# YuliangXiu/ICON

Measured on AMD Instinct MI355X. Metric: query-points/sec at 256^3 grid, higher is better.
Workload: dtype f32 via 3x f16 split MFMA (22-bit operands, f32 accumulate)

## Files before the change

### icon_amd/csrc/fused_f16x3.hip

```cpp
#pragma clang fp contract(off)

#include "geom_device.h"
#include "batch_device.h"
#include "mlp_f16x3_device.h"
#include "mlp_plain_device.h"

#include <algorithm>
#include <mutex>

namespace icon {

constexpr int kTilePts = kF16Pts;
constexpr int kXsOff = kSideOff + 4352;
constexpr int kFusedLds = kXsOff + kTilePts * kXRow * 4;

struct SignSrc {
    int mode;
    const int8_t *list;
    const int64_t *k_dev;
    int64_t k_host, rank_offset;
    const int8_t *gathered;
    int64_t stride;
    int world, rank;
    const int64_t *seg;
// ... 159 lines not shown
    const int planes = zb - za;
    if ((int)blockIdx.x < row_wgs) {
        const int64_t row = (int64_t)blockIdx.x * 256 + threadIdx.x;
        if (row >= (int64_t)planes * res) return;
        const int iy = (int)(row % res), iz = za + (int)(row / res);
        float *o = out + ((int64_t)(iz - z0) * res + iy) * res;
        o[0] = 0.0f; o[res - 1] = 0.0f;
        return;
    }
    const int f = ((int)blockIdx.x - row_wgs) * 4 + (int)(threadIdx.x >> 6);
    const int lane = threadIdx.x & 63;
    int iy, iz;
    if (f < 2 * planes) { iz = za + (f >> 1); iy = (f & 1) ? res - 1 : 0; }
    else {
        const int g = f - 2 * planes;
        const bool has0 = za == 0, has1 = zb == res;
        const int pl = g / res;
        if (pl >= (has0 ? 1 : 0) + (has1 ? 1 : 0)) return;
        iz = (pl == 0 && has0) ? 0 : res - 1;
        iy = g % res;
    }
    float *o = out + ((int64_t)(iz - z0) * res + iy) * res;
    for (int x = lane; x < res; x += 64) o[x] = 0.0f;
}

__device__ __forceinline__ float sign_at(const SignSrc &sg, int64_t mm)
{
    if (sg.mode == kSignSeg) {
        int r = 0;
        int64_t base = 0;
        for (int q = 1; q < sg.world; ++q) {
            const int64_t o = sg.seg[q];
            const bool ge = mm >= o;
            r += ge ? 1 : 0;
            base = ge ? o : base;
        }
        const int64_t e = mm - base;
        const uint32_t byte = (uint8_t)sg.gathered[(int64_t)r * sg.stride + 8 + (e >> 2)];
        return (float)((int)((byte >> (2 * (int)(e & 3))) & 3u) - 1);
    }
    return (float)sg.list[mm];
}

__device__ __forceinline__ int64_t lattice_item(const FusedGeom &G, int64_t q, int &ix, int &iy, int &iz)
{
    const uint32_t nx = (uint32_t)G.nx, qq = (uint32_t)q;
    const uint32_t r = qq / nx, lx = qq - r * nx, lz = r / nx, ly = r - lz * nx;
    ix = G.off + (int)lx; iy = G.off + (int)ly; iz = G.zs + (int)lz;
    return ((int64_t)(iz - G.z0) * G.res + iy) * G.res + ix;
}

__device__ __forceinline__ int64_t uniform64(int64_t v)
{
    const uint32_t lo = (uint32_t)__builtin_amdgcn_readfirstlane((int)(uint32_t)v);
    const uint32_t hi = (uint32_t)__builtin_amdgcn_readfirstlane((int)(uint32_t)((uint64_t)v >> 32));
    return (int64_t)(((uint64_t)hi << 32) | lo);
}

__device__ __forceinline__ void icon_row(const FusedGeom &G, const MeshDev &m, const FeatDev &f, f3 p, int64_t i, float *xrow, int64_t K, int64_t rank0)
{
    const uint32_t code = G.code8[i];
    Nearest nr;
    nr.slot = near_slot_of(G.near, i); nr.face = 0;
    nr.d2 = (code & kCodeOutlier) ? 0.0f : near_d2(G.near, i);
    const SdfOut o = sdf_attrs(m, p, nr, (code & kCodeInside) != 0);
    float s = o.sdf;
    f3 cmv = o.cm;
    if (code & kCodeOutlier) {
        s = (float)((int)((code >> kCodeSignShift) & 3u) - 1);
        if (G.cmap_local) cmv = mk3(s, s, s);
        else if (K > 0 && (f.smpl_mask & kSmplCmap)) {
            const int64_t blk = i >> 8;
            const int g = (int)(i >> 6) & 3;
            const unsigned long long *mk = G.grp_mask + blk * 4;
            int before = __popcll(mk[g] & ((1ull << (i & 63)) - 1ull));
            if (g > 0) before += __popcll(mk[0]);
            if (g > 1) before += __popcll(mk[1]);
            if (g > 2) before += __popcll(mk[2]);
            const int64_t jr = rank0 + G.block_offsets[blk] + before;
            float c3[3];
#pragma unroll
            for (int k = 0; k < 3; ++k) {
                int64_t mm = 3 * jr + k;
                if (mm >= K) mm -= K;
                if (mm >= K) mm -= K;
                c3[k] = sign_at(G.sg, mm);
            }
            cmv = mk3(c3[0], c3[1], c3[2]);
        }
    }
    gather_planes_dyn(f, (f.n_select == 2 && o.vis == 0.0f) ? 1 : 0, p.x, p.y, xrow);
    int hh = f.csel;
    xrow[hh++] = s;
    if (f.smpl_mask & kSmplCmap) { xrow[hh] = cmv.x; xrow[hh + 1] = cmv.y; xrow[hh + 2] = cmv.z; hh += 3; }
    if (f.smpl_mask & kSmplNorm) { xrow[hh] = o.nrm.x; xrow[hh + 1] = o.nrm.y; xrow[hh + 2] = o.nrm.z; }
    xrow[kCodeSlot] = __int_as_float((int)(code & kCodeInCube));
}

template <int PRIOR, Src SRC>
__device__ __forceinline__ void build_row(const FusedGeom &G, const BatchDev &bd, int64_t q, float *xrow, int64_t K, int64_t rank0)
{
    f3 p;
    int64_t i;
    const int64_t b = SRC == Src::Batch ? q / bd.n : 0;
    if (SRC == Src::Lattice) {
        int ix, iy, iz;
        i = lattice_item(G, q, ix, iy, iz);
        p = lattice_world(G.res, ix, iy, iz);
    } else {
        i = q;
        p = project(SRC == Src::Batch ? batch_calib(bd, b) : resolve_calib(G.cal), mk3(G.pts[3 * i], G.pts[3 * i + 1], G.pts[3 * i + 2]));
    }
    const FeatDev f = SRC == Src::Batch ? batch_feat(G.f, bd, b) : G.f;
    if (PRIOR == ICON_PRIOR_ICON) {
        icon_row(G, SRC == Src::Batch ? bd.meshes[b] : G.m, f, p, i, xrow, K, rank0);
    } else {
        gather_planes_dyn(f, 0, p.x, p.y, xrow);
        const int hh = f.csel;
        if (PRIOR == ICON_PRIOR_PAMIR) {
            float v[8];
            if (f.vpad == 8) gather_volume<2>(f, p.x, p.y, p.z, v); else gather_volume<1>(f, p.x, p.y, p.z, v);
#pragma unroll
            for (int k = 0; k < 8; ++k) if (k < f.Cv) xrow[hh + k] = v[k];
        } else {
            xrow[hh] = p.z;
        }
        xrow[kCodeSlot] = __int_as_float((int)in_cube_bit(p));
    }
}

__device__ __forceinline__ void sign_list_extent(const FusedGeom &G, int64_t &K, int64_t &rank0)
{
    K = 0; rank0 = 0;
    if (G.cmap_local) return;
    if (G.sg.mode == kSignSelf) K = *G.sg.k_dev;
    else if (G.sg.mode == kSignGlobal) { K = G.sg.k_host; rank0 = G.sg.rank_offset; }
    else if (G.sg.mode == kSignSeg) { K = G.sg.seg[G.sg.world]; rank0 = G.sg.seg[G.sg.rank]; }
}

template <int PRIOR, Src SRC, bool SMALL = false>
__global__ __launch_bounds__(kF16Block, 2) void k_fused_f16x3(FusedGeom G, float *__restrict__ out, MlpF16Dev w, BatchDev bd)
{
    extern __shared__ __attribute__((aligned(16))) char smem[];
    const int lane0 = threadIdx.x & 63, wave0 = __builtin_amdgcn_readfirstlane(threadIdx.x >> 6);
    float *Xs = reinterpret_cast<float *>(smem + kXsOff);
    if (G.clock && threadIdx.x == 0) {
        if (blockIdx.x == 0) wg_stamp(G.clock);
        if (blockIdx.x < kMaxProfGrid) wg_stamp(G.clock + 4 + kWgRec * blockIdx.x);
    }

    issue_units(w.image, smem + kW0Off, kW0Bytes / 1024, wave0, lane0);
    float *side = reinterpret_cast<float *>(smem + kSideOff);
    for (int i = threadIdx.x; i < kSideFloats; i += kF16Block) side[i] = w.side[i];
    const float *sb0 = side, *sb1 = side + 512, *sb2 = side + 768, *sw3 = side + kW3Float;
    int64_t K = 0, rank0 = 0;
    if (PRIOR == ICON_PRIOR_ICON) sign_list_extent(G, K, rank0);
    K = uniform64(K); rank0 = uniform64(rank0);

    if (SRC != Src::Batch && G.n_dev) { G.N = *G.n_dev; if (G.N <= 0) return; }
    const int tp = (SMALL && G.N <= (int64_t)(kTilePts / 2) * gridDim.x) ? kTilePts / 2 : kTilePts;
    const int ntiles = (int)((G.N + tp - 1) / tp);
    const bool stealing = !SMALL && G.steal != nullptr;
    const int per = ntiles / (int)gridDim.x, rem = ntiles % (int)gridDim.x;
    int tile = (int)blockIdx.x * per + min((int)blockIdx.x, rem);
    int tile_end = tile + (stealing ? min(G.steal_static, per) : per + ((int)blockIdx.x < rem ? 1 : 0));
    tile = __builtin_amdgcn_readfirstlane(tile);
    tile_end = __builtin_amdgcn_readfirstlane(tile_end);
    volatile int *pool = reinterpret_cast<volatile int *>(smem + kPoolOff);
    if (!SMALL) {
        if (threadIdx.x == 0) {
            pool[kPoolPer] = per; pool[kPoolRem] = rem; pool[kPoolStatic] = G.steal_static; pool[kPoolGroup] = G.steal_grp;
            pool[kPoolNGrp] = G.steal_ngrp; pool[kPoolGrid] = (int)gridDim.x; pool[kPoolDone] = 0; pool[kPoolMask] = 0; pool[kPoolNext] = -1;
            if (stealing && tile >= tile_end) pool_draw(G.steal, pool);
        }
        __syncthreads();
        if (stealing && tile >= tile_end) {
            const int word = __builtin_amdgcn_readfirstlane(pool[kPoolNext]);
            __syncthreads();
            if (word >= 0) { tile = word & ((1 << kPoolLenShift) - 1); tile_end = tile + (word >> kPoolLenShift); }
        }
    }
    if (tile < tile_end) issue_chunk(w.image, smem, 0, wave0, lane0);

    for (int nb = -1; tile < tile_end;) {
        int tid = threadIdx.x;
        asm volatile("" : "+v"(tid));
        const int lane = tid & 63, wave = __builtin_amdgcn_readfirstlane(tid >> 6);
        const int r = lane & 15, g = lane >> 4;
        const int t = tid;
        const bool draw = !SMALL && stealing && tile + 1 == tile_end;
        if (!SMALL && draw && t == 256) pool_draw(G.steal, pool);
        const bool worker = t < tp;
        int64_t q = (int64_t)tile * tp + (worker ? t : 0);
        if (q >= G.N) q = G.N - 1;
        if (worker) build_row<PRIOR, SRC>(G, bd, q, Xs + t * kXRow, K, rank0);
        __syncthreads();

        nb = (!SMALL && draw) ? __builtin_amdgcn_readfirstlane(pool[kPoolNext]) : -1;
        if (!SMALL && tid == 0) pool[kPoolDone] = pool[kPoolDone] + 1;
        const bool more = tile + 1 < tile_end || nb >= 0;
        if (SMALL && wave >= (tp >> 5)) {
            for (int c = 0; c < 16; ++c) {
                issue_chunk(w.image, smem + ((c + 1) & 1) * kBufBytes, c + 1, wave, lane);
                ICON_CHUNK_BARRIER();
            }
            issue_chunk(w.image, smem + kBufBytes, 17, wave, lane);
            ICON_CHUNK_BARRIER();
            issue_chunk(w.image, smem, 18, wave, lane);
            ICON_CHUNK_BARRIER();
            issue_chunk(w.image, smem + kBufBytes, 19, wave, lane);
            ICON_CHUNK_BARRIER();
            if (more) issue_chunk(w.image, smem, 0, wave, lane);
            ++tile;
            continue;
        }
        const int pt = wave * 32 + 16 * (g & 1) + r;
        half8 xb[2];
        const float tail = load_x(Xs + (wave * 32 + r) * kXRow + 8 * (g & 1), Xs + (wave * 32 + 16 + r) * kXRow + 8 * (g & 1), sw3, w.c0, g, xb);
        float maskf = (__float_as_int(Xs[pt * kXRow + kCodeSlot]) & (int)kCodeInCube) ? 1.0f : 0.0f;
        asm volatile("" : "+v"(maskf));

        f32x4 acc1[16][2];
#pragma unroll
        for (int m = 0; m < 16; ++m) acc1[m][0] = acc1[m][1] = *reinterpret_cast<const f32x4 *>(sb1 + m * 16 + 4 * g);
        half8 bh[2], bl[2];
        const LeakyK k0{w.inv0, w.p0, w.q0}, k1{w.inv1, w.p1, w.q1};
        {
            f32x4 h0[2][2];
            l0_tiles(smem + kW0Off, sb0, 0, xb, g, lane, h0);
            activate_split(h0[0][0], h0[0][1], h0[1][0], h0[1][1], k0, bh, bl);
        }
        f32x4 acc2[8][2];
        for (int c = 0; c < 15; ++c) {
            l01_chunk<false>(smem + (c & 1) * kBufBytes, smem + ((c + 1) & 1) * kBufBytes, smem + kW0Off, sb0, w.image, c, acc1, xb,
                             k0, g, lane, wave, bh, bl);
            ICON_CHUNK_BARRIER();
        }
        l01_chunk<true>(smem + kBufBytes, smem, smem + kW0Off, sb0, w.image, 15, acc1, xb, k0, g, lane, wave, bh, bl);
        ICON_CHUNK_BARRIER();
#pragma unroll
        for (int m2 = 0; m2 < 8; ++m2) acc2[m2][0] = acc2[m2][1] = *reinterpret_cast<const f32x4 *>(sb2 + m2 * 16 + 4 * g);
        activate_split(acc1[0][0], acc1[1][0], acc1[0][1], acc1[1][1], k1, bh, bl);
        l2_chunk<0>(smem, smem + kBufBytes, w.image, acc1, acc2, xb, k1, g, lane, wave, bh, bl);
        ICON_CHUNK_BARRIER();
        l2_chunk<1>(smem + kBufBytes, smem, w.image, acc1, acc2, xb, k1, g, lane, wave, bh, bl);
        ICON_CHUNK_BARRIER();
        l2_chunk<2>(smem, smem + kBufBytes, w.image, acc1, acc2, xb, k1, g, lane, wave, bh, bl);
        ICON_CHUNK_BARRIER();
        l2_chunk<3>(smem + kBufBytes, smem, w.image, acc1, acc2, xb, k1, g, lane, wave, bh, bl, more ? 0 : -1);

        float y2[2];
        {
            int tid_3 = threadIdx.x;
            asm volatile("" : "+v"(tid_3), "+v"(acc2[0][0]));
            l3_sum(sw3, acc2, tail, LeakyK{w.inv2, w.p2, w.q2}, w.b3, (tid_3 >> 4) & 3, y2);
        }
        int tid_o = threadIdx.x;
        asm volatile("" : "+v"(tid_o), "+v"(y2[0]), "+v"(y2[1]));
        const int g_o = (tid_o >> 4) & 3, pt_o = (tid_o >> 6) * 32 + 16 * (g_o & 1) + (tid_o & 15);
        const float y = apply_last_op(g_o == 0 ? y2[0] : y2[1], w.last_op);
        const int64_t oq = (int64_t)tile * tp + pt_o;
        if (g_o < 2 && oq < G.N) {
            int ix, iy, iz;
            out[SRC == Src::Lattice ? lattice_item(G, oq, ix, iy, iz) : ((SRC == Src::Points && G.out_map) ? (int64_t)G.out_map[oq] : oq)] = masked_result(y, maskf != 0.0f, w.flag);
        }
        if (!SMALL && nb >= 0) {
            tile = nb & ((1 << kPoolLenShift) - 1);
            tile_end = tile + (nb >> kPoolLenShift);
        } else ++tile;
    }
    if (!SMALL && stealing && threadIdx.x == 0) {
        __threadfence();
        if (atomicAdd(G.steal + 8, 1u) == gridDim.x - 1)
            for (int k = 0; k < 9; ++k) atomicExch(G.steal + k, 0u);
    }
    if (G.clock && threadIdx.x == 0 && blockIdx.x < kMaxProfGrid) {
        if (blockIdx.x == 0) wg_stamp(G.clock + 2);
        unsigned long long *rec = G.clock + 4 + kWgRec * blockIdx.x;
        wg_stamp(rec + 2);
        unsigned xcc, hw;
        asm volatile("s_getreg_b32 %0, hwreg(HW_REG_XCC_ID)" : "=s"(xcc));
        asm volatile("s_getreg_b32 %0, hwreg(HW_REG_HW_ID)" : "=s"(hw));
        rec[4] = ((unsigned long long)xcc << 32) | hw;
        rec[5] = SMALL ? 0ull : (unsigned long long)pool[kPoolDone];
    }
}

template <int PRIOR, Src SRC>
__global__ __launch_bounds__(64) void k_rescue_fused(FusedGeom G, float *__restrict__ out, MlpPlain P, const int *flag, int always, BatchDev bd)
{
    __shared__ float s[kPlainLds];
    if (!always && *flag == 0) return;
    if (SRC != Src::Batch && G.n_dev) G.N = *G.n_dev;
    const int lane = threadIdx.x;
    int64_t K = 0, rank0 = 0;
    if (PRIOR == ICON_PRIOR_ICON) sign_list_extent(G, K, rank0);
    for (int64_t base = (int64_t)blockIdx.x * 64; base < G.N; base += (int64_t)gridDim.x * 64) {
        const int64_t q = base + lane;
        int ix, iy, iz;
        const int64_t o = q < G.N ? (SRC == Src::Lattice ? lattice_item(G, q, ix, iy, iz) : ((SRC == Src::Points && G.out_map) ? (int64_t)G.out_map[q] : q)) : 0;
        const float v = q < G.N ? out[o] : 0.0f;
        unsigned long long todo = __ballot(not_finite(v));
        while (todo) {
            const int b = __ffsll((long long)todo) - 1;
            todo &= todo - 1;
            if (lane == b) {
                float row[kXRow];
#pragma unroll
                for (int k = 0; k < kXRow; ++k) row[k] = 0.0f;
                build_row<PRIOR, SRC>(G, bd, q, row, K, rank0);
#pragma unroll
                for (int k = 0; k < kXRow; ++k) s[k] = k < P.c0 ? row[k] : 0.0f;
            }
            const float y = mlp_plain_wave(P, s, lane);
            if (lane == b) out[o] = y;
            __builtin_amdgcn_wave_barrier();
        }
    }
}

__global__ void k_seg_offsets(const int8_t *__restrict__ gathered, int64_t stride, int world, int64_t *__restrict__ seg)
{
    if (threadIdx.x != 0 || blockIdx.x != 0) return;
    int64_t a = 0;
    for (int r = 0; r < world; ++r) { seg[r] = a; a += *reinterpret_cast<const int64_t *>(gathered + (int64_t)r * stride); }
    seg[world] = a;
}

int launch_sign(const icon_mesh *mesh, const Calib &cal, int res, int z0, const float *d_points, int64_t N, float sdf_clip,
                const icon_work *work, bool lattice, hipStream_t st, const BatchDev *bd)
{
    const int64_t nb = (N + 255) / 256;
    ICON_ARG(nb > 0 && nb < (1ll << 31), "too many workgroups for one launch");
    const float far_box2 = far_box_dist2(sdf_clip);
    if (lattice) hipLaunchKernelGGL(k_sign<true>, dim3((unsigned)nb), dim3(256), 0, st, mesh->dev, cal, res, z0, d_points, N, sdf_clip,
                                    work->d_row_count, work->d_row_slots, work_near(work, mesh), work->d_code8, work->d_block_counts,
                                    (unsigned long long *)work->d_grp_mask, far_box2, (const int *)nullptr, work->d_flag);
    else if (bd)
        hipLaunchKernelGGL(k_sign_wide<true>, dim3((unsigned)nb), dim3(1024), 0, st, MeshDev{}, Calib{}, d_points, N, sdf_clip, work_near(work, mesh), work->d_code8,
                           work->d_block_counts, (unsigned long long *)work->d_grp_mask, far_box2, (const int *)nullptr, work->d_flag, *bd);
    else if (work->q_n_dev || N <= 262144)
        hipLaunchKernelGGL(k_sign_wide<false>, dim3((unsigned)nb), dim3(1024), 0, st, mesh->dev, cal, d_points, N, sdf_clip, work_near(work, mesh), work->d_code8,
                           work->d_block_counts, (unsigned long long *)work->d_grp_mask, far_box2, work->q_n_dev, work->d_flag, BatchDev{});
    else hipLaunchKernelGGL(k_sign<false>, dim3((unsigned)nb), dim3(256), 0, st, mesh->dev, cal, res, z0, d_points, N, sdf_clip,
                            (const int32_t *)nullptr, (const int32_t *)nullptr, work_near(work, mesh), work->d_code8, work->d_block_counts,
                            (unsigned long long *)work->d_grp_mask, far_box2, work->q_n_dev, work->d_flag);
    ICON_HIP(hipGetLastError());
    work->flag_clean = work->d_flag != nullptr;
    return ICON_OK;
}

namespace {
constexpr int kMaxDevices = 64, kMaxKernelIds = 16;
std::mutex g_dev_mutex;
int g_n_cu[kMaxDevices];
bool g_attr_set[kMaxKernelIds][kMaxDevices];
}

int device_cu_count(int *n_cu)
{
    int dev = 0;
    ICON_HIP(hipGetDevice(&dev));
    ICON_ARG(dev >= 0 && dev < kMaxDevices, "device index out of range");
    std::lock_guard<std::mutex> lk(g_dev_mutex);
    if (!g_n_cu[dev]) {
        int n = 0;
        ICON_HIP(hipDeviceGetAttribute(&n, hipDeviceAttributeMultiprocessorCount, dev));
        g_n_cu[dev] = n > 0 ? n : 256;
    }
    *n_cu = g_n_cu[dev];
    return ICON_OK;
}

int once_per_device(int kernel_id, const std::function<hipError_t()> &set)
{
    int dev = 0;
    if (hipGetDevice(&dev) != hipSuccess || dev < 0 || dev >= kMaxDevices || kernel_id < 0 || kernel_id >= kMaxKernelIds) {
        const hipError_t e = set();
        return e == hipSuccess ? ICON_OK : fail(ICON_ERR_HIP, std::string("hipFuncSetAttribute: ") + hipGetErrorString(e));
    }
    std::lock_guard<std::mutex> lk(g_dev_mutex);
    if (g_attr_set[kernel_id][dev]) return ICON_OK;
    const hipError_t e = set();
    if (e != hipSuccess) return fail(ICON_ERR_HIP, std::string("hipFuncSetAttribute: ") + hipGetErrorString(e));
    g_attr_set[kernel_id][dev] = true;
    return ICON_OK;
}

int launch_fused_f16x3(const icon_mesh *mesh, const icon_feat *feat, const icon_mlp *mlp, int prior, const Calib &cal,
                       const LatticeMap &L, int za, int zb, const float *d_points, int64_t N, float sdf_clip, int cmap_local,
                       const icon_work *work, const FusedSigns &fs, float *d_occ, bool lattice, hipStream_t st, const BatchDev *bd)
{
    FusedGeom G{};
    if (mesh) G.m = mesh->dev;
    G.f = feat->dev; G.cal = cal; G.pts = d_points; G.sdf_clip = sdf_clip; G.cmap_local = cmap_local;
    if (lattice) {
        const int zs = std::max(za, L.off), ze = std::min(zb, L.res - L.off);
        if (L.off) {
            const int64_t rows = (int64_t)(zb - za) * L.res;
            const int row_wgs = (int)((rows + 255) / 256);
            const int64_t face_rows = 2 * (int64_t)(zb - za) + (int64_t)((za == 0 ? 1 : 0) + (zb == L.res ? 1 : 0)) * L.res;
            if (rows > 0) hipLaunchKernelGGL(k_shell_zero, dim3((unsigned)(row_wgs + (face_rows + 3) / 4)), dim3(256), 0, st, d_occ, L.res, L.z0, za, zb, row_wgs);
// ... 80 lines not shown
```

### icon_amd/csrc/mlp_f16x3.hip

```cpp
#include "mlp_f16x3_device.h"

#include <cmath>
#include <cstring>

namespace icon {

template <bool MASK>
__global__ __launch_bounds__(kF16Block, 2) void k_mlp_f16x3(const float *__restrict__ X, int64_t N, float *__restrict__ out, MlpF16Dev w)
{
    extern __shared__ __attribute__((aligned(16))) char smem[];
    const int lane = threadIdx.x & 63, wave = __builtin_amdgcn_readfirstlane(threadIdx.x >> 6);
    const int r = lane & 15, g = lane >> 4;
    const int64_t base = ((int64_t)blockIdx.x * (kF16Block / 64) + wave) * 32;
    const int64_t pi0 = min(base + r, N - 1), pi1 = min(base + 16 + r, N - 1);
    const int64_t po = (g & 1) ? pi1 : pi0;

    issue_units(w.image, smem + kW0Off, kW0Bytes / 1024, wave, lane);
    float *side = reinterpret_cast<float *>(smem + kSideOff);
    for (int i = threadIdx.x; i < kSideFloats; i += kF16Block) side[i] = w.side[i];
    const float *sb0 = side, *sb1 = side + 512, *sb2 = side + 768, *sw3 = side + kW3Float;

    float maskf = 1.0f;
    if (MASK) {
        const uint32_t code = (uint32_t)__float_as_int(X[po * kXRow + kCodeSlot]);
        maskf = (code & kCodeInCube) ? 1.0f : 0.0f;
        asm volatile("" : "+v"(maskf));
    }
    issue_chunk(w.image, smem, 0, wave, lane);
    __syncthreads();
    half8 xb[2];
    const float tail = load_x(X + pi0 * kXRow + 8 * (g & 1), X + pi1 * kXRow + 8 * (g & 1), sw3, w.c0, g, xb);

    f32x4 acc1[16][2];
#pragma unroll
    for (int m = 0; m < 16; ++m) acc1[m][0] = acc1[m][1] = *reinterpret_cast<const f32x4 *>(sb1 + m * 16 + 4 * g);

    half8 bh[2], bl[2];
    const LeakyK k0{w.inv0, w.p0, w.q0}, k1{w.inv1, w.p1, w.q1};
    {
        f32x4 h0[2][2];
        l0_tiles(smem + kW0Off, sb0, 0, xb, g, lane, h0);
        activate_split(h0[0][0], h0[0][1], h0[1][0], h0[1][1], k0, bh, bl);
    }
    for (int c = 0; c < 15; ++c) {
        l01_chunk<false>(smem + (c & 1) * kBufBytes, smem + ((c + 1) & 1) * kBufBytes, smem + kW0Off, sb0, w.image, c, acc1, xb,
                         k0, g, lane, wave, bh, bl);
        ICON_CHUNK_BARRIER();
    }
    l01_chunk<true>(smem + kBufBytes, smem, smem + kW0Off, sb0, w.image, 15, acc1, xb, k0, g, lane, wave, bh, bl);
    ICON_CHUNK_BARRIER();

    f32x4 acc2[8][2];
#pragma unroll
    for (int m2 = 0; m2 < 8; ++m2) acc2[m2][0] = acc2[m2][1] = *reinterpret_cast<const f32x4 *>(sb2 + m2 * 16 + 4 * g);
    activate_split(acc1[0][0], acc1[1][0], acc1[0][1], acc1[1][1], k1, bh, bl);
    l2_chunk<0>(smem, smem + kBufBytes, w.image, acc1, acc2, xb, k1, g, lane, wave, bh, bl);
    ICON_CHUNK_BARRIER();
    l2_chunk<1>(smem + kBufBytes, smem, w.image, acc1, acc2, xb, k1, g, lane, wave, bh, bl);
    ICON_CHUNK_BARRIER();
    l2_chunk<2>(smem, smem + kBufBytes, w.image, acc1, acc2, xb, k1, g, lane, wave, bh, bl);
    ICON_CHUNK_BARRIER();
    l2_chunk<3>(smem + kBufBytes, smem, w.image, acc1, acc2, xb, k1, g, lane, wave, bh, bl);

    float y2[2];
    {
        int tid_3 = threadIdx.x;
        asm volatile("" : "+v"(tid_3), "+v"(acc2[0][0]));
        l3_sum(sw3, acc2, tail, LeakyK{w.inv2, w.p2, w.q2}, w.b3, (tid_3 >> 4) & 3, y2);
    }
    int tid_o = threadIdx.x;
    asm volatile("" : "+v"(tid_o), "+v"(y2[0]), "+v"(y2[1]));
    const int g_o = (tid_o >> 4) & 3;
    const int64_t o = ((int64_t)blockIdx.x * (kF16Block / 64) + (tid_o >> 6)) * 32 + 16 * g_o + (tid_o & 15);
    const float y = apply_last_op(g_o == 0 ? y2[0] : y2[1], w.last_op);
    if (g_o < 2 && o < N) out[o] = masked_result(y, MASK ? maskf != 0.0f : true, w.flag);
}

uint16_t f32_to_f16_rtn(float f)
{
    uint32_t x; memcpy(&x, &f, 4);
    const uint32_t sign = (x >> 16) & 0x8000u;
    x &= 0x7fffffffu;
    if (x >= 0x7f800000u) return (uint16_t)(sign | 0x7c00u | (x > 0x7f800000u ? 0x200u : 0));
    if (x >= 0x477ff000u) return (uint16_t)(sign | 0x7c00u);
    if (x < 0x33000001u) return (uint16_t)sign;
    int e = (int)(x >> 23) - 127;
    uint32_t m = (x & 0x7fffffu) | 0x800000u;
    int shift;
    if (e < -14) { shift = 13 + (-14 - e); e = -15; } else shift = 13;
    uint32_t r = m >> shift;
    const uint32_t rem = m & ((1u << shift) - 1), half = 1u << (shift - 1);
    if (rem > half || (rem == half && (r & 1))) ++r;
    uint32_t out = (e == -15) ? r : (((uint32_t)(e + 15) << 10) + (r - 0x400u));
    return (uint16_t)(sign | out);
}

float f16_to_f32(uint16_t h)
{
    const uint32_t sign = (uint32_t)(h & 0x8000u) << 16;
    const int e = (h >> 10) & 31;
    const uint32_t m = h & 0x3ffu;
    float v;
    if (e == 0) v = std::ldexp((float)m, -24);
    else if (e == 31) v = m ? NAN : INFINITY;
    else v = std::ldexp((float)(m | 0x400u), e - 25);
    return sign ? -v : v;
}

float pick_scale(const std::vector<float> &W)
{
    float mx = 0.f;
    for (float v : W) mx = std::max(mx, std::fabs(v));
    if (!(mx > 0.f) || !std::isfinite(mx)) return 1.0f;
    int e = (int)std::floor(std::log2(8192.0 / (double)mx));
    e = std::min(std::max(e, -60), 60);
    return std::ldexp(1.0f, e);
}

float activation_scale(const std::vector<float> &W, const std::vector<float> &B, int cout, int cin, int n_used, const std::vector<double> &in_ms,
                       std::vector<double> &out_ms)
{
    out_ms.assign(cout, 0.0);
    double acc = 0.0;
    for (int c = 0; c < cout; ++c) {
        double s = (double)B[c] * B[c];
        for (int k = 0; k < n_used; ++k) s += (double)W[(size_t)c * cin + k] * W[(size_t)c * cin + k] * in_ms[k];
        out_ms[c] = s; acc += s;
    }
    const double typical = std::sqrt(acc / std::max(cout, 1));
    if (!(typical > 0.0) || !std::isfinite(typical)) return 1.0f;
    int e = (int)std::lround(std::log2(16.0 / typical));
    e = std::min(std::max(e, -60), 60);
    return std::ldexp(1.0f, e);
}

void mlp_pack_f16x3_host(int c0, const std::vector<std::vector<float>> &W, const std::vector<std::vector<float>> &B,
                         std::vector<uint16_t> &img, std::vector<float> &side, float inv[3], float scales[5])
{
    std::vector<double> ms_in(c0, 1.0), ms0, ms1;
    const float A0 = activation_scale(W[0], B[0], 512, c0, c0, ms_in, ms0);
    std::vector<float> W1(W[1]);
    for (float &v : W1) v /= A0;
    const float A1 = activation_scale(W[1], B[1], 256, 512, 512, ms0, ms1);
    const int ci2_ = 256 + c0;
    std::vector<float> W2(W[2]);
    for (int c = 0; c < 128; ++c)
        for (int k = 0; k < 256; ++k) W2[(size_t)c * ci2_ + k] /= A1;
    const float s0 = pick_scale(W[0]), s1 = pick_scale(W1), s2 = pick_scale(W2);
    img.assign(kImageBytes / 2, 0);
    auto sigma = [](int k) { const int g = k >> 3, e = k & 7; return e < 4 ? 4 * g + e : 16 + 4 * g + (e - 4); };
    auto put = [&](size_t at, size_t lo_step, float wv, float scale) {
        const float ws = wv * scale;
        const uint16_t hi = f32_to_f16_rtn(ws);
        img[at] = hi;
        img[at + lo_step] = f32_to_f16_rtn(ws - f16_to_f32(hi));
    };
    const int ci2 = 256 + c0;
    parallel_for(64, [&](int lane) {
        const int r = lane & 15, g = lane >> 4;
        for (int e = 0; e < 8; ++e) {
            const int ch = sigma(8 * g + e);
            const size_t col = (size_t)lane * 8 + e;
            for (int c = 0; c < 16; ++c)
                for (int mm = 0; mm < 16; ++mm)
                    put(((size_t)chunk_offset(c) + 2 * mm) * 512 + col, 512, W1[(size_t)(16 * mm + r) * 512 + 32 * c + ch], s1);
            for (int q = 0; q < 4; ++q)
                for (int mm = 0; mm < 2; ++mm)
                    for (int m2 = 0; m2 < 8; ++m2)
                        put(((size_t)chunk_offset(16 + q) + (mm * 8 + m2) * 2) * 512 + col, 512,
                            W2[(size_t)(16 * m2 + r) * ci2 + 32 * (2 * q + mm) + ch], s2);
        }
    });
    for (int g1 = 0; g1 < 2; ++g1)
        for (int r = 0; r < 16; ++r)
            for (int e = 0; e < 8; ++e) {
                const int k = 8 * g1 + e;
                const size_t col = (size_t)(g1 * 16 + r) * 8 + e;
                for (int ct = 0; ct < 32; ++ct)
                    put((size_t)ct * 512 + col, 256, k < c0 ? W[0][(size_t)(16 * ct + r) * c0 + k] : 0.f, s0);
                for (int m2 = 0; m2 < 8; ++m2)
                    put(((size_t)chunk_offset(16) + 32 + m2) * 512 + col, 256, k < c0 ? W2[(size_t)(16 * m2 + r) * ci2 + 256 + k] : 0.f, s2);
            }
    side.assign(kSideFloats, 0.f);
    float *b0 = side.data(), *b1 = b0 + 512, *b2 = b1 + 256, *w3 = side.data() + kW3Float;
    for (int c = 0; c < 512; ++c) b0[c] = B[0][c] * s0;
    for (int c = 0; c < 256; ++c) b1[c] = B[1][c] * s1;
    for (int c = 0; c < 128; ++c) b2[c] = B[2][c] * s2;
    for (int g = 0; g < 4; ++g) {
        for (int m2 = 0; m2 < 8; ++m2)
            for (int j = 0; j < 4; ++j) w3[g * kW3Stride + 4 * m2 + j] = W[3][16 * m2 + 4 * g + j];
        for (int s = 0; s < 8; ++s) w3[g * kW3Stride + 32 + s] = (s + 8 * (g & 1) < c0) ? W[3][128 + s + 8 * (g & 1)] : 0.f;
    }
    inv[0] = A0 / s0; inv[1] = A1 / s1; inv[2] = 1.0f / s2;
    scales[0] = s0; scales[1] = s1; scales[2] = s2; scales[3] = A0; scales[4] = A1;
}

int mlp_pack_f16x3(icon_mlp *m, const std::vector<std::vector<float>> &W, const std::vector<std::vector<float>> &B,
                   hipStream_t st)
{
    std::vector<uint16_t> img;
    std::vector<float> side;
    float scales[5];
    mlp_pack_f16x3_host(m->c0, W, B, img, side, m->f16_inv, scales);
    const size_t side_bytes = side.size() * sizeof(float);
    ICON_HIP(hipMalloc((void **)&m->d_f16, kImageBytes + side_bytes));
    ICON_HIP(hipMemcpyAsync(m->d_f16, img.data(), kImageBytes, hipMemcpyHostToDevice, st));
    ICON_HIP(hipMemcpyAsync(m->d_f16 + kImageBytes, side.data(), side_bytes, hipMemcpyHostToDevice, st));
    ICON_HIP(hipStreamSynchronize(st));
    return ICON_OK;
}

int mlp_launch_f16x3(const icon_mlp *mlp, const float *d_x, int64_t N, float *d_out, bool mask, hipStream_t st)
{
    if (N <= 0) return ICON_OK;
    MlpF16Dev w;
// ... 41 lines not shown
```

### icon_amd/csrc/mlp_f16x3_device.h

```cpp
#pragma once
#include "common.h"

namespace icon {

typedef float f32x4 __attribute__((ext_vector_type(4)));
typedef _Float16 half8 __attribute__((ext_vector_type(8)));
typedef __fp16 fp16x2 __attribute__((ext_vector_type(2)));
typedef __attribute__((address_space(1))) const void gvoid_t;
typedef __attribute__((address_space(3))) void lvoid_t;

constexpr int kF16Block = 512;
constexpr int kF16Pts = (kF16Block / 64) * 32;
constexpr int kBufBytes = 40 * 1024;
constexpr int kW3Stride = 40;
constexpr int kW3Float = 512 + 256 + 128;
constexpr int kZeroFloat = kW3Float + 4 * kW3Stride;
constexpr int kSideFloats = kZeroFloat + 4;
constexpr int kW0Off = 2 * kBufBytes;
constexpr int kW0Bytes = 32 * 1024;
constexpr int kSideOff = kW0Off + kW0Bytes;
constexpr int kLdsBytes = kSideOff + 4352;
constexpr int kZeroFromW0 = kSideOff + kZeroFloat * 4 - kW0Off;
constexpr int kZeroFromBuf0 = kSideOff + kZeroFloat * 4;
static_assert(kSideFloats * 4 <= 4352 && kZeroFromW0 % 16 == 0, "side arrays");

__host__ __device__ constexpr int chunk_units(int k) { return k == 16 ? 40 : 32; }
__host__ __device__ constexpr int chunk_offset(int k) { return 32 + 32 * k + (k > 16 ? 8 : 0); }
constexpr size_t kImageBytes = (size_t)(32 + 19 * 32 + 40) * 1024;

struct MlpF16Dev {
    const char *image;
    const float *side;
    float b3;
    float inv0, inv1, inv2;
    float p0, q0, p1, q1, p2, q2;
    int c0;
    int last_op;
    int *flag;
};

__device__ __forceinline__ float masked_result(float y, bool in_cube, int *flag)
{
    if (in_cube && not_finite(y)) *flag = 1;
    return in_cube ? y : 0.0f;
}

__device__ __forceinline__ fp16x2 residual_pair(fp16x2 hh, float v0, float v1)
{
    const int hb = __builtin_bit_cast(int, hh);
    int lb;
    asm("v_fma_mixlo_f16 %0, %1, -1.0, %2 op_sel_hi:[1,0,0]" : "=v"(lb) : "v"(hb), "v"(v0));
    asm("v_fma_mixhi_f16 %0, %1, -1.0, %2 op_sel:[1,0,0] op_sel_hi:[1,0,0]" : "+v"(lb) : "v"(hb), "v"(v1));
    return __builtin_bit_cast(fp16x2, lb);
}

__device__ __forceinline__ void split8(const float *v, half8 &hi, half8 &lo)
{
#pragma unroll
    for (int q = 0; q < 4; ++q) {
        const fp16x2 h = __builtin_amdgcn_cvt_pkrtz(v[2 * q], v[2 * q + 1]);
        const fp16x2 l = residual_pair(h, v[2 * q], v[2 * q + 1]);
        hi[2 * q] = (_Float16)h[0]; hi[2 * q + 1] = (_Float16)h[1];
        lo[2 * q] = (_Float16)l[0]; lo[2 * q + 1] = (_Float16)l[1];
    }
}

#ifndef ICON_ACT_EXACT
#define ICON_ACT_EXACT 0
#endif
struct LeakyK { float inv, p, q; };
__device__ __forceinline__ float leaky_scaled(float a, const LeakyK &k)
{
#if ICON_ACT_EXACT
    const float x = a * k.inv;
    return fmaxf(x, 0.01f * x);
#else
    return fmaf(fabsf(a), k.q, k.p * a);
#endif
}

#define MFMA32(a, b, c) __builtin_amdgcn_mfma_f32_16x16x32_f16((a), (b), (c), 0, 0, 0)

__device__ __forceinline__ half8 lds_op(const char *buf, int slot, int lane)
{
    return *reinterpret_cast<const half8 *>(buf + slot * 1024 + lane * 16);
}

#define ICON_CHUNK_BARRIER() __syncthreads()


__device__ __forceinline__ void issue_units(const char *src, char *buf, int units, int wave, int lane)
{
    for (int u = wave; u < units; u += kF16Block / 64)
        __builtin_amdgcn_global_load_lds((gvoid_t *)(src + u * 1024 + lane * 16), (lvoid_t *)(buf + u * 1024), 16, 0, 0);
}
__device__ __forceinline__ void issue_chunk(const char *image, char *buf, int k, int wave, int lane)
{
    issue_units(image + (size_t)chunk_offset(k) * 1024, buf, chunk_units(k), wave, lane);
}


#define GROUP6(ACC, M, AH, AL, BH, BL)                                                              \
    ACC[M][0] = MFMA32(AH, BH[0], ACC[M][0]); ACC[M][1] = MFMA32(AH, BH[1], ACC[M][1]);             \
    ACC[M][0] = MFMA32(AH, BL[0], ACC[M][0]); ACC[M][1] = MFMA32(AH, BL[1], ACC[M][1]);             \
    ACC[M][0] = MFMA32(AL, BH[0], ACC[M][0]); ACC[M][1] = MFMA32(AL, BH[1], ACC[M][1]);

__device__ __forceinline__ float load_x(const float *row0, const float *row1, const float *__restrict__ sw3, int c0, int g, half8 (&xb)[2])
{
    float tail = 0.0f;
#pragma unroll
    for (int b = 0; b < 2; ++b) {
        const float4 *q = reinterpret_cast<const float4 *>(b ? row1 : row0);
        const float4 u = q[0], v = q[1];
        float x[8] = {u.x, u.y, u.z, u.w, v.x, v.y, v.z, v.w};
#pragma unroll
        for (int s = 0; s < 8; ++s) x[s] = (s + 8 * (g & 1) < c0) ? x[s] : 0.0f;
        half8 hi, lo;
        split8(x, hi, lo);
        xb[b] = g < 2 ? hi : lo;
        float t = 0.0f;
#pragma unroll
        for (int s = 0; s < 8; ++s) t = fmaf(sw3[g * kW3Stride + 32 + s], x[s], t);
        tail = (g >> 1) == b ? t : tail;
    }
    asm volatile("" : "+v"(tail));
    return tail;
}

__device__ __forceinline__ void raw_operands(const char *__restrict__ base, int tile, int zero_off, int g, int lane, half8 &a1, half8 &a2)
{
    const int col = (lane & 31) * 16;
    const int lo_off = g < 2 ? 512 + col : zero_off, lo_mul = g < 2 ? 1024 : 0;
    a1 = *reinterpret_cast<const half8 *>(base + tile * 1024 + col);
    a2 = *reinterpret_cast<const half8 *>(base + lo_off + tile * lo_mul);
}

__device__ __forceinline__ void l0_tiles(const char *__restrict__ W0, const float *__restrict__ sb0, int c, const half8 (&xb)[2],
                                         int g, int lane, f32x4 (&h0)[2][2])
{
#pragma unroll
    for (int t = 0; t < 2; ++t) {
        const f32x4 bias = *reinterpret_cast<const f32x4 *>(sb0 + (2 * c + t) * 16 + 4 * g);
        half8 a1, a2;
        raw_operands(W0, 2 * c + t, kZeroFromW0, g, lane, a1, a2);
        h0[0][t] = MFMA32(a1, xb[0], bias); h0[1][t] = MFMA32(a1, xb[1], bias);
        h0[0][t] = MFMA32(a2, xb[0], h0[0][t]); h0[1][t] = MFMA32(a2, xb[1], h0[1][t]);
    }
}

__device__ __forceinline__ void act_part(const f32x4 &ta0, const f32x4 &tb0, const f32x4 &ta1, const f32x4 &tb1, int k, const LeakyK &inv,
                                         half8 (&nh)[2], half8 (&nl)[2])
{
    const int b = k >> 2, q = k & 3, j0 = (q & 1) * 2;
    const f32x4 &src = b ? (q >> 1 ? tb1 : ta1) : (q >> 1 ? tb0 : ta0);
    const float v0 = leaky_scaled(src[j0], inv), v1 = leaky_scaled(src[j0 + 1], inv);
    fp16x2 hh = __builtin_amdgcn_cvt_pkrtz(v0, v1);
    fp16x2 ll = residual_pair(hh, v0, v1);
    int hb = __builtin_bit_cast(int, hh), lb = __builtin_bit_cast(int, ll);
    asm volatile("" : "+v"(hb), "+v"(lb));
    hh = __builtin_bit_cast(fp16x2, hb); ll = __builtin_bit_cast(fp16x2, lb);
    nh[b][2 * q] = (_Float16)hh[0]; nh[b][2 * q + 1] = (_Float16)hh[1];
    nl[b][2 * q] = (_Float16)ll[0]; nl[b][2 * q + 1] = (_Float16)ll[1];
}

__device__ __forceinline__ void activate_split(const f32x4 &ta0, const f32x4 &tb0, const f32x4 &ta1, const f32x4 &tb1, const LeakyK &inv,
                                               half8 (&bh)[2], half8 (&bl)[2])
{
#pragma unroll
    for (int k = 0; k < 8; ++k) act_part(ta0, tb0, ta1, tb1, k, inv, bh, bl);
}

template <bool LAST>
__device__ __forceinline__ void l01_chunk(const char *__restrict__ L, char *__restrict__ nxt, const char *__restrict__ W0,
                                          const float *__restrict__ sb0, const char *image, int c, f32x4 (&acc1)[16][2],
                                          const half8 (&xb)[2], const LeakyK &inv0, int g4, int lane, int wave,
                                          half8 (&bh)[2], half8 (&bl)[2])
{
    issue_chunk(image, nxt, c + 1, wave, lane);
    f32x4 h0n[2][2];
    if (!LAST) l0_tiles(W0, sb0, c + 1, xb, g4, lane, h0n);
    half8 nh[2], nl[2];
    half8 a[2][2];
    a[0][0] = lds_op(L, 0, lane); a[0][1] = lds_op(L, 1, lane);
    __builtin_amdgcn_sched_barrier(0);
#pragma unroll
    for (int t = 0; t < 16; ++t) {
        if (t + 1 < 16) { a[(t + 1) & 1][0] = lds_op(L, 2 * t + 2, lane); a[(t + 1) & 1][1] = lds_op(L, 2 * t + 3, lane); }
        GROUP6(acc1, t, a[t & 1][0], a[t & 1][1], bh, bl)
        if (!LAST && (t & 1)) act_part(h0n[0][0], h0n[0][1], h0n[1][0], h0n[1][1], t >> 1, inv0, nh, nl);
        __builtin_amdgcn_sched_barrier(0);
    }
    if (!LAST) { bh[0] = nh[0]; bh[1] = nh[1]; bl[0] = nl[0]; bl[1] = nl[1]; }
}

template <int Q>
__device__ __forceinline__ void l2_chunk(const char *__restrict__ L, char *__restrict__ nxt, const char *image,
                                         f32x4 (&acc1)[16][2], f32x4 (&acc2)[8][2], const half8 (&xb)[2], const LeakyK &inv1,
                                         int g4, int lane, int wave, half8 (&bh)[2], half8 (&bl)[2], int next_chunk = (Q < 3) ? 17 + Q : -1)
{
    if (next_chunk >= 0) issue_chunk(image, nxt, next_chunk, wave, lane);
    if (Q == 0) {
#pragma unroll
        for (int m2 = 0; m2 < 8; ++m2) {
            half8 a1, a2;
            raw_operands(L, 32 + m2, kZeroFromBuf0, g4, lane, a1, a2);
            acc2[m2][0] = MFMA32(a1, xb[0], acc2[m2][0]); acc2[m2][1] = MFMA32(a1, xb[1], acc2[m2][1]);
            acc2[m2][0] = MFMA32(a2, xb[0], acc2[m2][0]); acc2[m2][1] = MFMA32(a2, xb[1], acc2[m2][1]);
        }
        __builtin_amdgcn_sched_barrier(0);
    }
#pragma unroll
    for (int mm = 0; mm < 2; ++mm) {
        constexpr int kLast = 7;
        const int kk = 2 * Q + mm, n = kk < kLast ? 2 * kk + 2 : 0;
        half8 nh[2], nl[2];
        half8 a[2][2];
        a[0][0] = lds_op(L, mm * 16, lane); a[0][1] = lds_op(L, mm * 16 + 1, lane);
        __builtin_amdgcn_sched_barrier(0);
#pragma unroll
        for (int t = 0; t < 8; ++t) {
            if (t + 1 < 8) { a[(t + 1) & 1][0] = lds_op(L, mm * 16 + 2 * t + 2, lane); a[(t + 1) & 1][1] = lds_op(L, mm * 16 + 2 * t + 3, lane); }
            GROUP6(acc2, t, a[t & 1][0], a[t & 1][1], bh, bl)
            if (kk < kLast) act_part(acc1[n][0], acc1[n + 1][0], acc1[n][1], acc1[n + 1][1], t, inv1, nh, nl);
            __builtin_amdgcn_sched_barrier(0);
        }
        if (kk < kLast) { bh[0] = nh[0]; bh[1] = nh[1]; bl[0] = nl[0]; bl[1] = nl[1]; }
    }
}

__device__ __forceinline__ void l3_sum(const float *__restrict__ sw3, const f32x4 (&acc2)[8][2], float tail, const LeakyK &inv2,
                                       float b3, int g, float (&y)[2])
{
    const float *w3 = sw3 + g * kW3Stride;
    float part[2] = {0.0f, 0.0f};
#pragma unroll
    for (int m2 = 0; m2 < 8; ++m2) {
        const f32x4 wv = *reinterpret_cast<const f32x4 *>(w3 + 4 * m2);
#pragma unroll
        for (int j = 0; j < 4; ++j) {
            part[0] = fmaf(wv[j], leaky_scaled(acc2[m2][0][j], inv2), part[0]);
            part[1] = fmaf(wv[j], leaky_scaled(acc2[m2][1][j], inv2), part[1]);
        }
    }
    const float t = tail + __shfl_xor(tail, 16);
    const float t_other = __shfl_xor(t, 32);
#pragma unroll
    for (int b = 0; b < 2; ++b) {
        part[b] += __shfl_xor(part[b], 16);
        part[b] += __shfl_xor(part[b], 32);
        y[b] = (part[b] + ((g >> 1) == b ? t : t_other)) + b3;
    }
}

}
```

Before: 1.096 billion.

## Restructure layer-1 loop with ping-pong buffers, fold biases into first MFMA

Layer 0/1 is rebuilt as an unroll-1 loop over chunk pairs. Ping-pong activation registers and compile-time buffer offsets (set through inline asm) replace the full unroll, with the aim of cutting code size, register pressure and per-iteration address arithmetic. Biases for layers 1 and 2 are now loaded as the initial accumulator of the first MFMA rather than pre-filled into all accumulators. The x-input masking in the fused kernel shrinks to a single slot, which relies on a one-time zero fill of the LDS X tile. The risks are scheduling changes from the non-unrolled loop and correctness for stale X columns.

```diff
diff --git a/icon_amd/csrc/fused_f16x3.hip b/icon_amd/csrc/fused_f16x3.hip
--- a/icon_amd/csrc/fused_f16x3.hip
+++ b/icon_amd/csrc/fused_f16x3.hip
@@ -335,7 +335,9 @@
     issue_units(w.image, smem + kW0Off, kW0Bytes / 1024, wave0, lane0);
     float *side = reinterpret_cast<float *>(smem + kSideOff);
     for (int i = threadIdx.x; i < kSideFloats; i += kF16Block) side[i] = w.side[i];
-    const float *sb0 = side, *sb1 = side + 512, *sb2 = side + 768, *sw3 = side + kW3Float;
+    const float *sb2 = side + 768, *sw3 = side + kW3Float;
+    for (int i = threadIdx.x; i < kTilePts * kXRow; i += kF16Block) Xs[i] = 0.0f;
+    __syncthreads();
     int64_t K = 0, rank0 = 0;
     if (PRIOR == ICON_PRIOR_ICON) sign_list_extent(G, K, rank0);
     K = uniform64(K); rank0 = uniform64(rank0);
@@ -399,38 +401,24 @@
         }
         const int pt = wave * 32 + 16 * (g & 1) + r;
         half8 xb[2];
-        const float tail = load_x(Xs + (wave * 32 + r) * kXRow + 8 * (g & 1), Xs + (wave * 32 + 16 + r) * kXRow + 8 * (g & 1), sw3, w.c0, g, xb);
+        const float tail = load_x<false>(Xs + (wave * 32 + r) * kXRow + 8 * (g & 1), Xs + (wave * 32 + 16 + r) * kXRow + 8 * (g & 1), sw3, w.c0, g, xb);
         float maskf = (__float_as_int(Xs[pt * kXRow + kCodeSlot]) & (int)kCodeInCube) ? 1.0f : 0.0f;
         asm volatile("" : "+v"(maskf));
 
         f32x4 acc1[16][2];
-#pragma unroll
-        for (int m = 0; m < 16; ++m) acc1[m][0] = acc1[m][1] = *reinterpret_cast<const f32x4 *>(sb1 + m * 16 + 4 * g);
+        const LeakyK k0{w.inv0, w.p0, w.q0}, k1{w.inv1, w.p1, w.q1};
+        l01_layer(smem, w.image, acc1, xb, k0, g, lane, wave);
+        ICON_CHUNK_BARRIER();
+        f32x4 acc2[8][2];
         half8 bh[2], bl[2];
-        const LeakyK k0{w.inv0, w.p0, w.q0}, k1{w.inv1, w.p1, w.q1};
-        {
-            f32x4 h0[2][2];
-            l0_tiles(smem + kW0Off, sb0, 0, xb, g, lane, h0);
-            activate_split(h0[0][0], h0[0][1], h0[1][0], h0[1][1], k0, bh, bl);
-        }
-        f32x4 acc2[8][2];
-        for (int c = 0; c < 15; ++c) {
-            l01_chunk<false>(smem + (c & 1) * kBufBytes, smem + ((c + 1) & 1) * kBufBytes, smem + kW0Off, sb0, w.image, c, acc1, xb,
-                             k0, g, lane, wave, bh, bl);
-            ICON_CHUNK_BARRIER();
-        }
-        l01_chunk<true>(smem + kBufBytes, smem, smem + kW0Off, sb0, w.image, 15, acc1, xb, k0, g, lane, wave, bh, bl);
+        activate_split(acc1[0][0], acc1[1][0], acc1[0][1], acc1[1][1], k1, bh, bl);
+        l2_chunk<0>(smem, smem + kBufBytes, w.image, sb2, acc1, acc2, xb, k1, g, lane, wave, bh, bl);
         ICON_CHUNK_BARRIER();
-#pragma unroll
-        for (int m2 = 0; m2 < 8; ++m2) acc2[m2][0] = acc2[m2][1] = *reinterpret_cast<const f32x4 *>(sb2 + m2 * 16 + 4 * g);
-        activate_split(acc1[0][0], acc1[1][0], acc1[0][1], acc1[1][1], k1, bh, bl);
-        l2_chunk<0>(smem, smem + kBufBytes, w.image, acc1, acc2, xb, k1, g, lane, wave, bh, bl);
+        l2_chunk<1>(smem, smem, w.image, sb2, acc1, acc2, xb, k1, g, lane, wave, bh, bl);
         ICON_CHUNK_BARRIER();
-        l2_chunk<1>(smem + kBufBytes, smem, w.image, acc1, acc2, xb, k1, g, lane, wave, bh, bl);
+        l2_chunk<2>(smem, smem + kBufBytes, w.image, sb2, acc1, acc2, xb, k1, g, lane, wave, bh, bl);
         ICON_CHUNK_BARRIER();
-        l2_chunk<2>(smem, smem + kBufBytes, w.image, acc1, acc2, xb, k1, g, lane, wave, bh, bl);
-        ICON_CHUNK_BARRIER();
-        l2_chunk<3>(smem + kBufBytes, smem, w.image, acc1, acc2, xb, k1, g, lane, wave, bh, bl, more ? 0 : -1);
+        l2_chunk<3>(smem, smem, w.image, sb2, acc1, acc2, xb, k1, g, lane, wave, bh, bl, more ? 0 : -1);
 
         float y2[2];
         {
diff --git a/icon_amd/csrc/mlp_f16x3.hip b/icon_amd/csrc/mlp_f16x3.hip
--- a/icon_amd/csrc/mlp_f16x3.hip
+++ b/icon_amd/csrc/mlp_f16x3.hip
@@ -18,7 +18,7 @@
     issue_units(w.image, smem + kW0Off, kW0Bytes / 1024, wave, lane);
     float *side = reinterpret_cast<float *>(smem + kSideOff);
     for (int i = threadIdx.x; i < kSideFloats; i += kF16Block) side[i] = w.side[i];
-    const float *sb0 = side, *sb1 = side + 512, *sb2 = side + 768, *sw3 = side + kW3Float;
+    const float *sb2 = side + 768, *sw3 = side + kW3Float;
 
     float maskf = 1.0f;
     if (MASK) {
@@ -29,38 +29,23 @@
     issue_chunk(w.image, smem, 0, wave, lane);
     __syncthreads();
     half8 xb[2];
-    const float tail = load_x(X + pi0 * kXRow + 8 * (g & 1), X + pi1 * kXRow + 8 * (g & 1), sw3, w.c0, g, xb);
+    const float tail = load_x<true>(X + pi0 * kXRow + 8 * (g & 1), X + pi1 * kXRow + 8 * (g & 1), sw3, w.c0, g, xb);
 
     f32x4 acc1[16][2];
-#pragma unroll
-    for (int m = 0; m < 16; ++m) acc1[m][0] = acc1[m][1] = *reinterpret_cast<const f32x4 *>(sb1 + m * 16 + 4 * g);
-
+    const LeakyK k0{w.inv0, w.p0, w.q0}, k1{w.inv1, w.p1, w.q1};
+    l01_layer(smem, w.image, acc1, xb, k0, g, lane, wave);
+    ICON_CHUNK_BARRIER();
+
+    f32x4 acc2[8][2];
     half8 bh[2], bl[2];
-    const LeakyK k0{w.inv0, w.p0, w.q0}, k1{w.inv1, w.p1, w.q1};
-    {
-        f32x4 h0[2][2];
-        l0_tiles(smem + kW0Off, sb0, 0, xb, g, lane, h0);
-        activate_split(h0[0][0], h0[0][1], h0[1][0], h0[1][1], k0, bh, bl);
-    }
-    for (int c = 0; c < 15; ++c) {
-        l01_chunk<false>(smem + (c & 1) * kBufBytes, smem + ((c + 1) & 1) * kBufBytes, smem + kW0Off, sb0, w.image, c, acc1, xb,
-                         k0, g, lane, wave, bh, bl);
-        ICON_CHUNK_BARRIER();
-    }
-    l01_chunk<true>(smem + kBufBytes, smem, smem + kW0Off, sb0, w.image, 15, acc1, xb, k0, g, lane, wave, bh, bl);
-    ICON_CHUNK_BARRIER();
-
-    f32x4 acc2[8][2];
-#pragma unroll
-    for (int m2 = 0; m2 < 8; ++m2) acc2[m2][0] = acc2[m2][1] = *reinterpret_cast<const f32x4 *>(sb2 + m2 * 16 + 4 * g);
     activate_split(acc1[0][0], acc1[1][0], acc1[0][1], acc1[1][1], k1, bh, bl);
-    l2_chunk<0>(smem, smem + kBufBytes, w.image, acc1, acc2, xb, k1, g, lane, wave, bh, bl);
-    ICON_CHUNK_BARRIER();
-    l2_chunk<1>(smem + kBufBytes, smem, w.image, acc1, acc2, xb, k1, g, lane, wave, bh, bl);
-    ICON_CHUNK_BARRIER();
-    l2_chunk<2>(smem, smem + kBufBytes, w.image, acc1, acc2, xb, k1, g, lane, wave, bh, bl);
-    ICON_CHUNK_BARRIER();
-    l2_chunk<3>(smem + kBufBytes, smem, w.image, acc1, acc2, xb, k1, g, lane, wave, bh, bl);
+    l2_chunk<0>(smem, smem + kBufBytes, w.image, sb2, acc1, acc2, xb, k1, g, lane, wave, bh, bl);
+    ICON_CHUNK_BARRIER();
+    l2_chunk<1>(smem, smem, w.image, sb2, acc1, acc2, xb, k1, g, lane, wave, bh, bl);
+    ICON_CHUNK_BARRIER();
+    l2_chunk<2>(smem, smem + kBufBytes, w.image, sb2, acc1, acc2, xb, k1, g, lane, wave, bh, bl);
+    ICON_CHUNK_BARRIER();
+    l2_chunk<3>(smem, smem, w.image, sb2, acc1, acc2, xb, k1, g, lane, wave, bh, bl);
 
     float y2[2];
     {
diff --git a/icon_amd/csrc/mlp_f16x3_device.h b/icon_amd/csrc/mlp_f16x3_device.h
--- a/icon_amd/csrc/mlp_f16x3_device.h
+++ b/icon_amd/csrc/mlp_f16x3_device.h
@@ -86,6 +86,14 @@
     return *reinterpret_cast<const half8 *>(buf + slot * 1024 + lane * 16);
 }
 
+template <int BOFF>
+__device__ __forceinline__ int buffer_base(int lane)
+{
+    int vo = lane * 16;
+    if (BOFF) asm volatile("v_add_u32 %0, %1, %2" : "=v"(vo) : "n"(BOFF), "v"(lane * 16));
+    return vo;
+}
+
 #define ICON_CHUNK_BARRIER() __syncthreads()
 
 
@@ -104,7 +112,11 @@
     ACC[M][0] = MFMA32(AH, BH[0], ACC[M][0]); ACC[M][1] = MFMA32(AH, BH[1], ACC[M][1]);             \
     ACC[M][0] = MFMA32(AH, BL[0], ACC[M][0]); ACC[M][1] = MFMA32(AH, BL[1], ACC[M][1]);             \
     ACC[M][0] = MFMA32(AL, BH[0], ACC[M][0]); ACC[M][1] = MFMA32(AL, BH[1], ACC[M][1]);
-
+#define GROUP4(ACC, M, AH, AL, BH, BL)                                                              \
+    ACC[M][0] = MFMA32(AH, BL[0], ACC[M][0]); ACC[M][1] = MFMA32(AH, BL[1], ACC[M][1]);             \
+    ACC[M][0] = MFMA32(AL, BH[0], ACC[M][0]); ACC[M][1] = MFMA32(AL, BH[1], ACC[M][1]);
+
+template <bool MASK_ALL>
 __device__ __forceinline__ float load_x(const float *row0, const float *row1, const float *__restrict__ sw3, int c0, int g, half8 (&xb)[2])
 {
     float tail = 0.0f;
@@ -113,8 +125,12 @@
         const float4 *q = reinterpret_cast<const float4 *>(b ? row1 : row0);
         const float4 u = q[0], v = q[1];
         float x[8] = {u.x, u.y, u.z, u.w, v.x, v.y, v.z, v.w};
-#pragma unroll
-        for (int s = 0; s < 8; ++s) x[s] = (s + 8 * (g & 1) < c0) ? x[s] : 0.0f;
+        if (MASK_ALL) {
+#pragma unroll
+            for (int s = 0; s < 8; ++s) x[s] = (s + 8 * (g & 1) < c0) ? x[s] : 0.0f;
+        } else {
+            x[kCodeSlot & 7] = ((g & 1) && c0 <= kCodeSlot) ? 0.0f : x[kCodeSlot & 7];
+        }
         half8 hi, lo;
         split8(x, hi, lo);
         xb[b] = g < 2 ? hi : lo;
@@ -135,14 +151,24 @@
     a2 = *reinterpret_cast<const half8 *>(base + lo_off + tile * lo_mul);
 }
 
-__device__ __forceinline__ void l0_tiles(const char *__restrict__ W0, const float *__restrict__ sb0, int c, const half8 (&xb)[2],
-                                         int g, int lane, f32x4 (&h0)[2][2])
+struct L0Addr {
+    int bias;
+    int a1;
+    int a2, a2_mul;
+};
+__device__ __forceinline__ L0Addr l0_addr(int g, int lane)
+{
+    const int col = (lane & 31) * 16;
+    return L0Addr{kSideOff + 16 * g, kW0Off + col, g < 2 ? kW0Off + 512 + col : kZeroFromBuf0, g < 2 ? 1024 : 0};
+}
+
+__device__ __forceinline__ void l0_tiles(const char *__restrict__ S, const L0Addr &at, int d, const half8 (&xb)[2], f32x4 (&h0)[2][2])
 {
 #pragma unroll
     for (int t = 0; t < 2; ++t) {
-        const f32x4 bias = *reinterpret_cast<const f32x4 *>(sb0 + (2 * c + t) * 16 + 4 * g);
-        half8 a1, a2;
-        raw_operands(W0, 2 * c + t, kZeroFromW0, g, lane, a1, a2);
+        const f32x4 bias = *reinterpret_cast<const f32x4 *>(S + at.bias + (d + t) * 64);
+        const half8 a1 = *reinterpret_cast<const half8 *>(S + at.a1 + (d + t) * 1024);
+        const half8 a2 = *reinterpret_cast<const half8 *>(S + at.a2 + (d + t) * at.a2_mul);
         h0[0][t] = MFMA32(a1, xb[0], bias); h0[1][t] = MFMA32(a1, xb[1], bias);
         h0[0][t] = MFMA32(a2, xb[0], h0[0][t]); h0[1][t] = MFMA32(a2, xb[1], h0[1][t]);
     }
@@ -170,41 +196,79 @@
     for (int k = 0; k < 8; ++k) act_part(ta0, tb0, ta1, tb1, k, inv, bh, bl);
 }
 
-template <bool LAST>
-__device__ __forceinline__ void l01_chunk(const char *__restrict__ L, char *__restrict__ nxt, const char *__restrict__ W0,
-                                          const float *__restrict__ sb0, const char *image, int c, f32x4 (&acc1)[16][2],
-                                          const half8 (&xb)[2], const LeakyK &inv0, int g4, int lane, int wave,
-                                          half8 (&bh)[2], half8 (&bl)[2])
-{
+enum { kChunkFirst = 0, kChunkMid = 1, kChunkLast = 2 };
+template <int KIND, int BOFF>
+__device__ __forceinline__ void l01_chunk(const char *__restrict__ S, char *__restrict__ nxt, const char *image, int c, const L0Addr &at,
+                                          int d, f32x4 (&acc1)[16][2], const half8 (&xb)[2], const LeakyK &inv0, int lane, int wave,
+                                          const half8 (&bh)[2], const half8 (&bl)[2], half8 (&nh)[2], half8 (&nl)[2])
+{
+    constexpr bool FIRST = KIND == kChunkFirst, LAST = KIND == kChunkLast;
     issue_chunk(image, nxt, c + 1, wave, lane);
     f32x4 h0n[2][2];
-    if (!LAST) l0_tiles(W0, sb0, c + 1, xb, g4, lane, h0n);
-    half8 nh[2], nl[2];
+    if (!LAST) l0_tiles(S, at, d, xb, h0n);
+    const char *L = S + buffer_base<BOFF>(lane);
     half8 a[2][2];
-    a[0][0] = lds_op(L, 0, lane); a[0][1] = lds_op(L, 1, lane);
+    f32x4 bias[2];
+    a[0][0] = lds_op(L, 0, 0); a[0][1] = lds_op(L, 1, 0);
+    if (FIRST) bias[0] = *reinterpret_cast<const f32x4 *>(S + at.bias + 2048);
     __builtin_amdgcn_sched_barrier(0);
 #pragma unroll
     for (int t = 0; t < 16; ++t) {
-        if (t + 1 < 16) { a[(t + 1) & 1][0] = lds_op(L, 2 * t + 2, lane); a[(t + 1) & 1][1] = lds_op(L, 2 * t + 3, lane); }
-        GROUP6(acc1, t, a[t & 1][0], a[t & 1][1], bh, bl)
+        if (t + 1 < 16) {
+            a[(t + 1) & 1][0] = lds_op(L, 2 * t + 2, 0); a[(t + 1) & 1][1] = lds_op(L, 2 * t + 3, 0);
+            if (FIRST) bias[(t + 1) & 1] = *reinterpret_cast<const f32x4 *>(S + at.bias + 2048 + (t + 1) * 64);
+        }
+        if (FIRST) {
+            acc1[t][0] = MFMA32(a[t & 1][0], bh[0], bias[t & 1]); acc1[t][1] = MFMA32(a[t & 1][0], bh[1], bias[t & 1]);
+            GROUP4(acc1, t, a[t & 1][0], a[t & 1][1], bh, bl)
+        } else {
+            GROUP6(acc1, t, a[t & 1][0], a[t & 1][1], bh, bl)
+        }
         if (!LAST && (t & 1)) act_part(h0n[0][0], h0n[0][1], h0n[1][0], h0n[1][1], t >> 1, inv0, nh, nl);
         __builtin_amdgcn_sched_barrier(0);
     }
-    if (!LAST) { bh[0] = nh[0]; bh[1] = nh[1]; bl[0] = nl[0]; bl[1] = nl[1]; }
-}
-
-template <int Q>
-__device__ __forceinline__ void l2_chunk(const char *__restrict__ L, char *__restrict__ nxt, const char *image,
+}
+
+constexpr int kL1Pairs = 7;
+__device__ __forceinline__ void l01_layer(char *smem, const char *image, f32x4 (&acc1)[16][2], const half8 (&xb)[2], const LeakyK &k0,
+                                          int g, int lane, int wave)
+{
+    char *const buf0 = smem, *const buf1 = smem + kBufBytes;
+    L0Addr at = l0_addr(g, lane);
+    half8 ah[2], al[2], bh[2], bl[2];
+    {
+        f32x4 h0[2][2];
+        l0_tiles(smem, at, 0, xb, h0);
+        activate_split(h0[0][0], h0[0][1], h0[1][0], h0[1][1], k0, ah, al);
+    }
+    l01_chunk<kChunkFirst, 0>(smem, buf1, image, 0, at, 2, acc1, xb, k0, lane, wave, ah, al, bh, bl);
+    ICON_CHUNK_BARRIER();
+#pragma unroll 1
+    for (int p = 0; p < kL1Pairs; ++p) {
+        at.bias += 4 * 64; at.a1 += 4 * 1024; at.a2 += 4 * at.a2_mul;
+        asm volatile("" : "+v"(at.bias), "+v"(at.a1), "+v"(at.a2));
+        l01_chunk<kChunkMid, kBufBytes>(smem, buf0, image, 2 * p + 1, at, 0, acc1, xb, k0, lane, wave, bh, bl, ah, al);
+        ICON_CHUNK_BARRIER();
+        l01_chunk<kChunkMid, 0>(smem, buf1, image, 2 * p + 2, at, 2, acc1, xb, k0, lane, wave, ah, al, bh, bl);
+        ICON_CHUNK_BARRIER();
+    }
+    l01_chunk<kChunkLast, kBufBytes>(smem, buf0, image, 15, at, 0, acc1, xb, k0, lane, wave, bh, bl, ah, al);
+}
+
+template <int Q, int BOFF = (Q & 1) * kBufBytes>
+__device__ __forceinline__ void l2_chunk(const char *__restrict__ S, char *__restrict__ nxt, const char *image, const float *__restrict__ sb2,
                                          f32x4 (&acc1)[16][2], f32x4 (&acc2)[8][2], const half8 (&xb)[2], const LeakyK &inv1,
                                          int g4, int lane, int wave, half8 (&bh)[2], half8 (&bl)[2], int next_chunk = (Q < 3) ? 17 + Q : -1)
 {
     if (next_chunk >= 0) issue_chunk(image, nxt, next_chunk, wave, lane);
+    const char *L = S + buffer_base<BOFF>(lane);
     if (Q == 0) {
 #pragma unroll
         for (int m2 = 0; m2 < 8; ++m2) {
+            const f32x4 bias = *reinterpret_cast<const f32x4 *>(sb2 + m2 * 16 + 4 * g4);
             half8 a1, a2;
-            raw_operands(L, 32 + m2, kZeroFromBuf0, g4, lane, a1, a2);
-            acc2[m2][0] = MFMA32(a1, xb[0], acc2[m2][0]); acc2[m2][1] = MFMA32(a1, xb[1], acc2[m2][1]);
+            raw_operands(S, 32 + m2, kZeroFromBuf0, g4, lane, a1, a2);
+            acc2[m2][0] = MFMA32(a1, xb[0], bias); acc2[m2][1] = MFMA32(a1, xb[1], bias);
             acc2[m2][0] = MFMA32(a2, xb[0], acc2[m2][0]); acc2[m2][1] = MFMA32(a2, xb[1], acc2[m2][1]);
         }
         __builtin_amdgcn_sched_barrier(0);
@@ -215,11 +279,11 @@
         const int kk = 2 * Q + mm, n = kk < kLast ? 2 * kk + 2 : 0;
         half8 nh[2], nl[2];
         half8 a[2][2];
-        a[0][0] = lds_op(L, mm * 16, lane); a[0][1] = lds_op(L, mm * 16 + 1, lane);
+        a[0][0] = lds_op(L, mm * 16, 0); a[0][1] = lds_op(L, mm * 16 + 1, 0);
         __builtin_amdgcn_sched_barrier(0);
 #pragma unroll
         for (int t = 0; t < 8; ++t) {
-            if (t + 1 < 8) { a[(t + 1) & 1][0] = lds_op(L, mm * 16 + 2 * t + 2, lane); a[(t + 1) & 1][1] = lds_op(L, mm * 16 + 2 * t + 3, lane); }
+            if (t + 1 < 8) { a[(t + 1) & 1][0] = lds_op(L, mm * 16 + 2 * t + 2, 0); a[(t + 1) & 1][1] = lds_op(L, mm * 16 + 2 * t + 3, 0); }
             GROUP6(acc2, t, a[t & 1][0], a[t & 1][1], bh, bl)
             if (kk < kLast) act_part(acc1[n][0], acc1[n + 1][0], acc1[n][1], acc1[n + 1][1], t, inv1, nh, nl);
             __builtin_amdgcn_sched_barrier(0);
```

After: 1.094 billion. No clear change (-0.2%).
